# Genesis-Embodied-AI/ThinShellLab

Hardware: AMD Instinct MI355X
Metric: element-steps/s (fwd+adjoint), 100k-tri cloth; 1/2/4/8-GPU scaling (higher is better)
Workload: dtype f64

## Files before the change

### thinshelllab_amd/context.py

```python
import ctypes as C
import os

import numpy as np
import torch

from . import _lib
from ._lib import Body, ClothDesc, ContactPair, ElasticDesc, SceneDesc, SolveStats, StepStats, check


def _np(a, dt):
    return np.ascontiguousarray(a, dtype=dt)


def _ptr(t):
    if t is None:
        return None
    if isinstance(t, torch.Tensor):
        assert t.is_contiguous(), "tensor must be contiguous"
        return C.c_void_p(t.data_ptr())
    return C.c_void_p(t.ctypes.data)


def scene_desc(*, tot_NV, dt, mass, gravity, frozen, cloths=(), elastics=(), faces=None, bodies=(), pairs=(),
               k_contact=1000.0, eps_contact=1e-3, eps_v=0.01, damping=1.0, max_n_constraints=10000, grid_h=0.003, device=None):
# ... 591 lines not shown
        check(self.L.tsl_profile_read_events(self.h, C.byref(ev)), "tsl_profile_read_events")
        return dict(ms_per_launch=ms.value, launches=n.value, bytes_per_launch=b.value, ms_per_launch_events=ev.value)

    def bench_direct(self, cls, reps=20):
        out = (C.c_double * 4)()
        check(self.L.tsl_bench_direct(self.h, int(cls), int(reps), out), "tsl_bench_direct")
        return dict(us_per_launch=out[0], flops_per_launch=out[1], bytes_per_launch=out[2], launches=int(out[3]))

    def direct_info(self):
        out = (C.c_double * 10)()
        check(self.L.tsl_direct_info(self.h, out), "tsl_direct_info")
        keys = ("plans", "factorizations", "applications", "perturbed_pivots", "plan_seconds", "supernodes", "levels", "batches", "flops_per_factorization", "front_bytes")
        return dict(zip(keys, [float(v) for v in out]))

    def direct_counters(self):
        out = (C.c_double * 13)()
        check(self.L.tsl_direct_counters(self.h, out, 13), "tsl_direct_counters")
        keys = ("flow_launches", "flow_aborts", "plan_cache_hits", "panel_bytes", "schur_bytes", "g_bytes", "schur_entries", "plans_parked",
                "berr_seen", "berr_accepted", "berr_max", "berr_rel_max", "tiles_guarded")
        return dict(zip(keys, [float(v) for v in out]))

    def bench_spmv(self, variant=20, reps=500):
        us = C.c_double(0)
        check(self.L.tsl_bench_spmv(self.h, int(variant), int(reps), C.byref(us)), "tsl_bench_spmv")
        return us.value
```

### thinshelllab_amd/csrc/direct_host.hpp

```cpp
#pragma once
#include <array>
#include <chrono>

#include "k_direct.hpp"
#include "tsl_ctx.hpp"

#include <cerrno>
#include <fcntl.h>
#include <sys/file.h>
#include <sys/stat.h>
#include <unistd.h>
static void ds_flow_token_acquire(DirectSolver& d) {
  char bus[64] = "dev";
  if (hipDeviceGetPCIBusId(bus, sizeof(bus), d.device) != hipSuccess) { (void)hipGetLastError(); snprintf(bus, sizeof(bus), "dev%d", d.device); }
  for (char* q = bus; *q; q++) if (*q == ':' || *q == '/') *q = '_';
  d.flow_token = -1; d.flow_token_asked = d.n_factor;
  for (const char* dir : {"/dev/shm", "/tmp"}) {
    const std::string path = std::string(dir) + "/tsl_flow_" + bus;
    int fd = open(path.c_str(), O_RDWR | O_CLOEXEC);
    if (fd < 0 && errno == ENOENT) {
      fd = open(path.c_str(), O_CREAT | O_RDWR | O_CLOEXEC, 0666);
      if (fd < 0 && (errno == ENOENT || errno == ENOTDIR)) continue;
      if (fd < 0 && errno == EEXIST) fd = open(path.c_str(), O_RDWR | O_CLOEXEC);
    } else if (fd < 0 && errno == ENOTDIR) continue;
// ... 9 lines not shown
  d.flow_token_fd = -1; d.flow_token = 0;
}
static bool ds_flow_token_held(DirectSolver& d) {
  if (d.token_lender) return ds_flow_token_held(*d.token_lender);
  if (d.flow_token == 0 || (d.flow_token < 0 && d.n_factor - d.flow_token_asked >= 256)) ds_flow_token_acquire(d);
  return d.flow_token > 0;
}

static inline int ds_nblk(long n, int b) { return (int)((n + b - 1) / b); }

static inline bool ds_use_small(const DirectSolver& d, const DsBatch& b) {
  if (b.max_pp > DS_SMALL) return false;
  return (size_t)b.count <= (size_t)d.plan.n_cu * ds_small_per_cu(b.max_pp) * (size_t)d.small_rounds;
}

static void ds_launch_gemm(hipStream_t s, const DsDev& D, const DsBatch& b, int mode, int ds_xcd_map, int ds_g32_below = 0, int part = 0, int max_lead = 0) {
  const int rows = mode == 0 ? b.max_pp : b.max_bp, cols = b.max_bp;
  const dim3 grid((cols + 63) / 64, (rows + 63) / 64, b.count);
  const long tiles = (long)grid.x * grid.y * grid.z;
  const int ta = (max_lead + 63) / 64;
  if (part == 1 && ta == 0) return;
  if (mode == 1 && part != 0) {
    hipLaunchKernelGGL((k_ds_gemm<1, 4>), part == 1 ? dim3(ta, ta, b.count) : grid, dim3(256), 0, s, D, b.first, part);
    return;
  }
  if (mode == 0 && ds_g32_below > 0 && tiles < ds_g32_below) {
    hipLaunchKernelGGL(k_ds_gemm_g32, dim3(part == 1 ? 2 * ta : (cols + 31) / 32, (rows + 31) / 32, b.count), dim3(256), 0, s, D, b.first, part);
    return;
  }
  if (mode == 0 && part != 0) {
    hipLaunchKernelGGL((k_ds_gemm<0, 4>), part == 1 ? dim3(ta, grid.y, b.count) : grid, dim3(256), 0, s, D, b.first, part);
    return;
  }
  if (ds_xcd_map > 0 && b.count >= ds_xcd_map) {
    const int gx = grid.x, gy = grid.y, nf = b.count;
    const long ng = ((long)nf + 7) / 8 * 8 * gx * gy;
    if (mode == 0) hipLaunchKernelGGL((k_ds_gemm_x<0, 4>), dim3((unsigned)ng), dim3(256), 0, s, D, b.first, gx, gy, nf);
    else hipLaunchKernelGGL((k_ds_gemm_x<1, 4>), dim3((unsigned)ng), dim3(256), 0, s, D, b.first, gx, gy, nf);
    return;
  }
  if (mode == 0) hipLaunchKernelGGL((k_ds_gemm<0, 4>), grid, dim3(256), 0, s, D, b.first, 0);
  else hipLaunchKernelGGL((k_ds_gemm<1, 4>), grid, dim3(256), 0, s, D, b.first, 0);
}
static void ds_launch_extend(hipStream_t s, const DsDev& D, int lv0, int nf, int max_ld, int part = 0, int max_span = 0) {
  const int xspan = part == 1 ? 64 * DS_XU : DS_XSPAN;
  const int nsp = ((part == 0 ? max_ld : max_span) + xspan - 1) / xspan;
  if (nsp <= 0) return;
  hipLaunchKernelGGL(k_ds_extend_panels, dim3(((max_ld / 3 + 2 + 3) / 4) * nsp, nf), dim3(256), 0, s, D, lv0, nsp, part, xspan);
}
static void ds_launch_level_start(tsl_ctx* c, hipStream_t s, const DsDev& D, int l, int part = 0, const DsBatch* b = nullptr) {
  DirectSolver& d = c->ds;
  const DirectPlan& P = d.plan;
  const int lv0 = P.level_ptr[l], nf = P.level_ptr[l + 1] - lv0;
  if (l > 0) ds_launch_extend(s, D, lv0, nf, P.level_maxld[l], part, part == 0 ? 0 : part == 1 ? b->max_pp : std::max(b->max_bp, b->max_pp));
  const int i0 = part == 2 ? P.blk_lmid[l] : P.blk_lptr[l], i1 = part == 1 ? P.blk_lmid[l] : P.blk_lptr[l + 1];
  const int nb = i1 - i0, npad = part == 2 ? 0 : nf;
  const long nt = (long)nb * 9 + (long)npad * DS_T;
  if (nt > 0)
    hipLaunchKernelGGL(k_ds_assemble_level, dim3(ds_nblk(nt, 256)), dim3(256), 0, s, i0, nb, (const int*)d.blk_q.p, (const double*)c->vals.p, (const long long*)d.blk_dst.p,
                       (const int*)d.blk_ld.p, lv0, npad, d.frl.p, d.arena.p, l == 0 ? 1 : 0);
  if (c->nc > 0) {
    const int g0 = part == 2 ? P.cgr_lmid[l] : P.cgr_lptr[l], g1 = part == 1 ? P.cgr_lmid[l] : P.cgr_lptr[l + 1];
    const int ng = g1 - g0;
    if (ng > 0) hipLaunchKernelGGL(k_ds_assemble_contacts_level, dim3(ds_nblk((long)ng * 64, 256)), dim3(256), 0, s, g0, ng, (const int*)d.cgr_ptr.p, (const int*)d.cgr_ent.p,
                                   (const long long*)d.cgr_dst.p, (const int*)d.cgr_ld.p, (const double*)c->c_H.p, d.arena.p);
  }
}


static long ds_flow_wgs(const DirectPlan& P, const DsBatch& b) {
  long n = 0;
  for (int z = 0; z < b.count; z++) { const long ns = (P.fr[P.level_sn[b.first + z]].pp / DS_T + DS_FLOW_B - 1) / DS_FLOW_B; n += ns * ns; }
  return n;
}
static bool ds_flow_eligible(DirectSolver& d, const DirectPlan& P, const DsBatch& b, hipStream_t s) {
  if (!d.flow || b.count > DS_FLOW_MAXF || b.max_pp < 2 * DS_T) return false;
  { hipStreamCaptureStatus cs = hipStreamCaptureStatusNone;
    if (hipStreamIsCapturing(s, &cs) != hipSuccess || cs != hipStreamCaptureStatusNone) return false; }
  if (!ds_flow_token_held(d)) return false;
  if (ds_use_small(d, b) && !(d.flow & 2)) return false;
  if (d.flow_cap == 0) {
    int occ = 0, dev = 0;
    hipDeviceProp_t prop;
// ... 325 lines not shown
static int direct_factor(tsl_ctx* c, int stop_sn = -1, const char* dump_path = nullptr, const double* eager_r = nullptr, double* eager_z = nullptr) {
  DirectSolver& d = c->ds;
  hipStream_t s = c->stream;
  TSL_TRY(direct_plan(c));
  if (d.numeric_valid) return 0;
  d.eager_n = 0;
  const DirectPlan& P = d.plan;
  const DsDev D = ds_dev(c);
  if (d.prezero_pending) {
    HIP_OK(hipStreamWaitEvent(s, d.ev_zero, 0));
    d.prezero_pending = false;
    if (P.leaf_ranges.empty() && d.prezero_n < (size_t)P.arena_leaf) HIP_OK(hipMemsetAsync(d.arena.p + d.prezero_n, 0, ((size_t)P.arena_leaf - d.prezero_n) * sizeof(double), s));
  } else if (P.leaf_ranges.empty()) HIP_OK(hipMemsetAsync(d.arena.p, 0, (size_t)P.arena_leaf * sizeof(double), s));
  else for (const auto& r : P.leaf_ranges) HIP_OK(hipMemsetAsync(d.arena.p + r.first, 0, (size_t)r.second * sizeof(double), s));
  HIP_OK(hipMemsetAsync(d.bad.p, 0, 8 * sizeof(int), s));
  bool swept_at_root = false;
  int flow_wgs_sent = 0;
  auto invert_batch = [&](const DsBatch& b, hipStream_t bs, bool& flow_free) {
    const int lv0 = b.first, nf = b.count;
    const int tp = b.max_pp / DS_T;
    bool flowed = false;
    {
      const std::vector<DsBatch> pieces = ds_flow_pieces(d, P, b, flow_free, bs);
      std::vector<DsFlowArgs> fas(pieces.size());
      bool ready = !pieces.empty();
      for (size_t i = 0; ready && i < pieces.size(); i++) ready = ds_flow_prepare(d, P, pieces[i], true, fas[i], bs);
      if (ready) {
        for (size_t i = 0; i < pieces.size(); i++) { ds_flow_launch(bs, D, pieces[i].first, fas[i], d); d.n_flow++; flow_wgs_sent += fas[i].tile0[fas[i].nf]; }
        flowed = true; flow_free = false;
      }
// ... 57 lines not shown
        const int c0 = std::min((d.lookahead >> 2) & 7, top - 2);
        const int c1r = (d.lookahead >> 5) & 15, c1 = c1r == 0 ? top - 1 : std::min(std::max(c1r, c0), top - 1);
        const int stage = lvl - (top - 2);
        const int lo = stage == 0 ? 0 : stage == 1 ? c0 : c1, hi = stage == 0 ? c0 : stage == 1 ? c1 : (c1r == 0 ? c1 : top);
        if (hi > lo && lo == d.eager_n && (stage > 0 || P.la_from < lvl)) {
          hipLaunchKernelGGL(k_ds_flow_gate, dim3(1), dim3(64), 0, ls, (const int*)(d.bad.p + DS_FLOW_ARRIVE), flow_wgs_sent);
          for (int l = lo; l < hi; l++) ds_sweep_up_level(ls, D, d, l, eager_r, eager_z);
          d.eager_n = hi; d.eager_r = eager_r; d.eager_z = eager_z;
          if (stage == 2) { HIP_OK(hipEventRecord(d.ev_la[LA_DRAIN], ls)); swept_at_root = true; }
        }
      }
      if (la_in) HIP_OK(hipStreamWaitEvent(s, d.ev_la[LA_REST], 0));
      if (b.max_bp > 0 && be < P.batches.size()) {
        int max_lead = 0;
        for (int q = 0; q < b.count; q++) max_lead = std::max(max_lead, P.fr[P.level_sn[b.first + q]].lead);
        HIP_OK(hipEventRecord(d.ev_la[LA_W], s));
        ds_launch_gemm(s, D, b, 0, 0, d.g32_below, 1, max_lead);
        HIP_OK(hipEventRecord(d.ev_la[LA_GA], s));
        ds_launch_gemm(s, D, b, 1, 0, 0, 1, max_lead);
        HIP_OK(hipEventRecord(d.ev_la[LA_A], s));
        HIP_OK(hipStreamWaitEvent(ls, d.ev_la[LA_W], 0));
        ds_launch_gemm(ls, D, b, 0, 0, d.g32_below, 2, max_lead);
        HIP_OK(hipStreamWaitEvent(ls, d.ev_la[LA_GA], 0));
        ds_launch_gemm(ls, D, b, 1, 0, 0, 2, max_lead);
      } else if (b.max_bp > 0) {
        ds_launch_gemm(s, D, b, 0, d.xcd_map, d.g32_below);
        ds_launch_gemm(s, D, b, 1, d.xcd_map);
      }
      bi = be;
      continue;
    }
    if (stop_here) {
      const DsFrontDesc& f = P.fr[stop_sn];
      std::vector<double> h((size_t)f.pp * f.ld);
// ... 217 lines not shown
```

### thinshelllab_amd/csrc/k_direct.hpp

```cpp
#pragma once
#include "direct_plan.hpp"
#include "tsl_device.hpp"

typedef double ds_d4 __attribute__((ext_vector_type(4)));

struct DsDev {
  const DsFrontDesc* fr;
  const DsFrontDesc* frl;
  const int* level_sn;
  double* A;
  double* S;
  double* G;
  double* scr;
  double* Y;
  const DsChildRec* ch;
  const int* pmap;
  const int* vtx;
  int* bad;
  double piv_tol;
  int dbg;
  unsigned long long* tlog;
};

__global__ void k_ds_rownorm(int NV, const int* __restrict__ slice_off, const int* __restrict__ slice_len, const double* __restrict__ vals, double* out) {
// ... 26 lines not shown
  if (t < (long)nblk * 9) {
    const long i = i0 + t / 9;
    const int e = (int)(t % 9);
    double* a = &A[dst[i] + (long long)(e / 3) * dld[i] + e % 3];
    const double v = vals[(size_t)src[i] + 64 * e];
    *a = cleared ? 0.0 + v : *a + v;
    return;
  }
  t -= (long)nblk * 9;
  if (t < (long)nf * DS_T) {
    const DsFrontDesc f = frl[lv0 + t / DS_T];
    const int i = f.p + (int)(t % DS_T);
    if (i < f.pp) A[f.off + (long long)i * f.ld + i] = 1.0;
  }
}
__global__ void __launch_bounds__(256) k_ds_assemble_contacts_level(int g0, int ng, const int* __restrict__ gptr, const int* __restrict__ gent, const long long* __restrict__ gdst,
                                                                    const int* __restrict__ gld, const double* __restrict__ H, double* __restrict__ A) {
  const int gi = (int)((blockIdx.x * (size_t)blockDim.x + threadIdx.x) >> 6), lane = threadIdx.x & 63;
  if (gi >= ng) return;
  const int g = g0 + gi;
  double v[9] = {0, 0, 0, 0, 0, 0, 0, 0, 0};
  for (int k = gptr[g] + lane; k < gptr[g + 1]; k += 64) {
    const int x = gent[k], c = x >> 4, sub = x & 15;
    const double* Hb = H + (size_t)c * 144 + (3 * (sub >> 2)) * 12 + 3 * (sub & 3);
#pragma unroll
    for (int r = 0; r < 3; r++)
#pragma unroll
      for (int cc = 0; cc < 3; cc++) v[3 * r + cc] += Hb[12 * r + cc];
  }
#pragma unroll
  for (int e = 0; e < 9; e++) v[e] = wave_sum(v[e]);
  if (lane == 0) {
    double* dst = A + gdst[g];
    const int ld = gld[g];
#pragma unroll
    for (int r = 0; r < 3; r++)
#pragma unroll
      for (int cc = 0; cc < 3; cc++) dst[(long long)r * ld + cc] += v[3 * r + cc];
  }
}

#define DS_PB 4
#define DS_BADLOG 64
#define DS_BAD_NOTE (8 + 4 * DS_BADLOG)
#define DS_BAD_INTS (DS_BAD_NOTE + 8)
#define DS_REDO 6
// ... 785 lines not shown
            }
      }
    }
    __syncthreads();
  }
  for (int i = ty; i < pp; i += 32) {
#pragma unroll
    for (int a = 0; a < 4; a++)
#pragma unroll
      for (int b = 0; b < 4; b++) if (b < nt) A[(size_t)(i + 8 * a) * f.ld + tx + 32 * b] = M[(i + 8 * a) * ls + tx + 32 * b];
  }
}

#define DS_SK 32
#define DS_GMC 8
template <int mode, int WPC>
TSL_DEV void ds_gemm_tile(const DsDev& D, int lv0, int bx, int by, int bz, int part = 0) {
  constexpr int SA = DS_SK + 1, SB = 64 + 1;
  __shared__ double As[64 * SA];
  __shared__ double Bs[DS_SK * SB];
  const DsFrontDesc f = D.frl[lv0 + bz];
  const int Mr = mode == 0 ? f.pp : f.bp, Nc = f.bp, K = f.pp;
  const int I0 = by * 64, J0 = bx * 64;
  if (I0 >= Mr || J0 >= Nc) return;
  if (mode == 1 && part != 0 && ((I0 < f.lead && J0 < f.lead) != (part == 1))) return;
  if (mode == 0 && part != 0 && ((J0 < f.lead) != (part == 1))) return;
  const double* F = D.A + f.off;
  double* G = D.G + f.goff;
  const int ld = f.ld, pp = f.pp;
  const double* Am = mode == 0 ? F : D.A + f.off21;
// ... 13 lines not shown
  double pa[8], pb0[4], pb1[4];
  auto gload = [&](int k0) {
#pragma unroll
    for (int q = 0; q < 8; q++) {
      const int r = ty + 8 * q;
      pa[q] = (r < 32 || rows_hi) ? Am[(size_t)(I0 + r) * lda + k0 + tx] : 0.0;
    }
#pragma unroll
    for (int q = 0; q < 4; q++) {
      const int r = ty + 8 * q;
      pb0[q] = Bm[(size_t)(k0 + r) * ldb + J0 + tx];
      pb1[q] = cols_hi ? Bm[(size_t)(k0 + r) * ldb + J0 + 32 + tx] : 0.0;
    }
  };
  gload(0);
  constexpr int GMC = DS_GMC;
  __shared__ int s_map[mode == 1 ? GMC : 1][128];
  __shared__ long long s_soff[mode == 1 ? GMC : 1];
  __shared__ int s_cbp[mode == 1 ? GMC : 1];
  int pre[GMC / 2];
  auto map_load = [&](int q) {
    const int k = threadIdx.x & 127;
    const int idx = k < 64 ? I0 + k : J0 + k - 64;
    return idx < f.bp ? D.pmap[D.ch[f.ch_off + q].pmap_off + pp + idx] : -1;
  };
  if (mode == 1) {
#pragma unroll
    for (int h = 0; h < GMC / 2; h++) { const int q = 2 * h + (threadIdx.x >> 7); pre[h] = q < f.nchild ? map_load(q) : -1; }
  }
  for (int k0 = 0; k0 < K; k0 += DS_SK) {
#pragma unroll
    for (int q = 0; q < 8; q++) As[(ty + 8 * q) * SA + tx] = pa[q];
#pragma unroll
    for (int q = 0; q < 4; q++) { Bs[(ty + 8 * q) * SB + tx] = pb0[q]; Bs[(ty + 8 * q) * SB + tx + 32] = pb1[q]; }
    __syncthreads();
    if (k0 + DS_SK < K) gload(k0 + DS_SK);
#pragma unroll
    for (int kk = 0; kk < DS_SK / 4; kk++) {
      const double a0 = As[(32 * wi + lr) * SA + 4 * kk + lk], a1 = As[(32 * wi + 16 + lr) * SA + 4 * kk + lk];
      const double b0 = Bs[(4 * kk + lk) * SB + 32 * wj + lr], b1 = Bs[(4 * kk + lk) * SB + 32 * wj + 16 + lr];
      acc[0][0] = __builtin_amdgcn_mfma_f64_16x16x4f64(a0, b0, acc[0][0], 0, 0, 0);
      acc[0][1] = __builtin_amdgcn_mfma_f64_16x16x4f64(a0, b1, acc[0][1], 0, 0, 0);
      acc[1][0] = __builtin_amdgcn_mfma_f64_16x16x4f64(a1, b0, acc[1][0], 0, 0, 0);
      acc[1][1] = __builtin_amdgcn_mfma_f64_16x16x4f64(a1, b1, acc[1][1], 0, 0, 0);
    }
    __syncthreads();
  }
  if (mode == 0) {
#pragma unroll
    for (int a = 0; a < 2; a++)
#pragma unroll
      for (int b = 0; b < 2; b++)
#pragma unroll
        for (int r = 0; r < 4; r++) {
          const int row = I0 + 32 * wi + 16 * a + lk + 4 * r, col = J0 + 32 * wj + 16 * b + lr;
          if (row < Mr && col < Nc) G[(size_t)row * f.bp + col] = acc[a][b][r];
        }
    return;
  }
  if (f.parent < 0) return;
  double s22[2][2][4];
#pragma unroll
  for (int a = 0; a < 2; a++)
#pragma unroll
    for (int b = 0; b < 2; b++)
#pragma unroll
      for (int r = 0; r < 4; r++) s22[a][b][r] = -acc[a][b][r];
  const int row0 = I0 + 32 * wi + lk, col0 = J0 + 32 * wj + lr;
  for (int q0 = 0; q0 < f.nchild; q0 += GMC) {
    const int nq = min(GMC, f.nchild - q0);
    if (q0 > 0) __syncthreads();
#pragma unroll
    for (int h = 0; h < GMC / 2; h++) {
      const int q = 2 * h + (threadIdx.x >> 7);
      if (q < nq) s_map[q][threadIdx.x & 127] = q0 == 0 ? pre[h] : map_load(q0 + q);
    }
    if ((int)threadIdx.x < nq) { const DsChildRec c = D.ch[f.ch_off + q0 + threadIdx.x]; s_soff[threadIdx.x] = c.soff; s_cbp[threadIdx.x] = c.bp; }
    __syncthreads();
    for (int q = 0; q < nq; q++) {
      const double* Sc = D.S + s_soff[q];
      const int cbp = s_cbp[q];
      const int cj0 = s_map[q][64 + 32 * wj + lr], cj1 = s_map[q][64 + 32 * wj + 16 + lr];
      const int dj0 = max(cj0, 0), dj1 = max(cj1, 0);
      int ci[2][4];
      double v0[2][4], v1[2][4];
#pragma unroll
      for (int a = 0; a < 2; a++)
#pragma unroll
        for (int r = 0; r < 4; r++) ci[a][r] = s_map[q][32 * wi + 16 * a + lk + 4 * r];
#pragma unroll
      for (int a = 0; a < 2; a++)
#pragma unroll
        for (int r = 0; r < 4; r++) {
          const double* Srow = Sc + (size_t)max(ci[a][r], 0) * cbp;
          v0[a][r] = Srow[dj0]; v1[a][r] = Srow[dj1];
        }
#pragma unroll
      for (int a = 0; a < 2; a++)
#pragma unroll
        for (int r = 0; r < 4; r++) {
          s22[a][0][r] = (ci[a][r] >= 0 && cj0 >= 0) ? s22[a][0][r] + v0[a][r] : s22[a][0][r];
          s22[a][1][r] = (ci[a][r] >= 0 && cj1 >= 0) ? s22[a][1][r] + v1[a][r] : s22[a][1][r];
        }
    }
  }
  double* Sf = D.S + f.soff;
#pragma unroll
  for (int a = 0; a < 2; a++)
#pragma unroll
    for (int r = 0; r < 4; r++) {
      const int row = row0 + 16 * a + 4 * r;
      if (row >= f.b) continue;
#pragma unroll
      for (int b = 0; b < 2; b++) {
        const int col = col0 + 16 * b;
        if (col < f.b) Sf[(size_t)row * f.bp + col] = s22[a][b][r];
      }
    }
}

#define DS_XU 4
#define DS_XSPAN 1024
#define DS_XMAXC 64
__global__ void __launch_bounds__(256) k_ds_extend_panels(DsDev D, int lv0, int nsp, int part, int xspan) {
  const DsFrontDesc f = D.frl[lv0 + blockIdx.y];
  const int ib = blockIdx.x / nsp, sp = blockIdx.x - ib * nsp;
  const int lane = threadIdx.x & 63, w = __builtin_amdgcn_readfirstlane(threadIdx.x >> 6);
  const int g = 4 * ib + w, ng = f.nv_own + f.nv_bnd;
  if (g >= ng + 2) return;
  const bool top = g >= ng ? g == ng : g < f.nv_own;
  if (!top && part == 1) return;
  const int ncol = top ? f.ld : f.pp;
  const int cA = (top && part == 2) ? f.pp : 0, cB = (top && part == 1) ? f.pp : ncol;
// ... 129 lines not shown
  for (int r = 0; r < 4; r++) G[(size_t)(I0 + 16 * wi + lk + 4 * r) * f.bp + J0 + 16 * wj + lr] = acc[r];
}

template <int mode, int WPC>
__global__ void __launch_bounds__(256, WPC) k_ds_gemm(DsDev D, int lv0, int part) {
  ds_gemm_tile<mode, WPC>(D, lv0, blockIdx.x, blockIdx.y, blockIdx.z, part);
}

template <int mode, int WPC>
__global__ void __launch_bounds__(256, WPC) k_ds_gemm_x(DsDev D, int lv0, int gx, int gy, int nf) {
  const unsigned L = blockIdx.x, xcd = L & 7, k = L >> 3;
  const unsigned tpf = (unsigned)gx * gy;
  const unsigned bz = (k / tpf) * 8 + xcd, t = k % tpf;
  if (bz >= (unsigned)nf) return;
  ds_gemm_tile<mode, WPC>(D, lv0, t % gx, t / gx, bz);
}

#define DS_VCHUNK 2048
TSL_DEV double ds_child_sum(const DsDev& D, const DsFrontDesc& f, int d) {
  int ci[4];
#pragma unroll
  for (int q = 0; q < 4; q++) ci[q] = q < f.nchild ? D.pmap[f.cpm[q] + d] : -1;
  double y[4];
#pragma unroll
  for (int q = 0; q < 4; q++) y[q] = ci[q] >= 0 ? D.Y[f.cy[q] + ci[q]] : 0.0;
  double a = ((y[0] + y[1]) + y[2]) + y[3];
  for (int q = 4; q < f.nchild; q++) {
    const DsChildRec c = D.ch[f.ch_off + q];
    const int cq = D.pmap[c.pmap_off + d];
    if (cq >= 0) a += D.Y[c.yoff + cq];
// ... 94 lines not shown
```

### thinshelllab_amd/csrc/tsl_ctx.hpp

```cpp
#pragma once
#include <memory>
#include <hip/hip_runtime.h>
#include <stdint.h>

#include <algorithm>
#include <cmath>
#include <cstdio>
#include <cstring>
#include <string>
#include <vector>

#include "../../include/tsl_hip.h"
#include "collider_host.hpp"
#include "sphere_host.hpp"
#include "box_host.hpp"
#include "sdf_host.hpp"
#include "capsule_host.hpp"
#include "k_body.hpp"
#include "direct_plan.hpp"
#include "scene_tables.hpp"

#define TSL_SLICE 64

extern thread_local std::string g_tsl_err;
// ... 91 lines not shown
  int eager_n = 0; const double* eager_r = nullptr; double* eager_z = nullptr;
  int lookahead = 103;
  int device = 0;
  int flow_wgs_last = 0;
  int flow = 3, flow_cap = 0, flow_epoch = 0;
  int flow_token = 0, flow_token_fd = -1;
  long flow_token_asked = 0;
  int small_rounds = 2;
  int xcd_map = 64;
  long n_flow = 0, n_flow_abort = 0;
  DevBuf<double> flow_x;
  DevBuf<int> flow_f;
  DevBuf<unsigned long long> tlog;
  int gemv_wide_below = 300;
  int g32_below = 1100;
  bool cons_checked = false;
  double* h_anorm = nullptr;
  int bench_batch = -1;
  double piv_tol = 1e-11;
  int fallback_cap = 1000;
  int leaf = 64;
  bool static_ready = false, numeric_valid = false;
  bool have_factor = false;
  int dbg = 0;
  double berr_tol = 1e-12, berr_rel_cap = 50.0;
  long berr_seen = 0, berr_accepted = 0;
  double berr_max = 0, berr_rel_max = 0;
  int n_setup_fail = 0;
  std::vector<std::unique_ptr<DsPlanSlot>> cache;
  int cache_cap = 64, cache_mb = 1024;
// ... 300 lines not shown
```

### thinshelllab_amd/csrc/tsl_hip.hip

```cpp
#include <stdarg.h>
#include <cctype>
#include <chrono>
#include <mutex>

#include <array>
#include <map>

#include "k_cloth.hpp"
#include "k_contact.hpp"
#include "k_fem.hpp"
#include "k_mg.hpp"
#include "k_param.hpp"
#include "k_solver.hpp"
#include "param_keys.hpp"
#include "tsl_ctx.hpp"

thread_local std::string g_tsl_err;
int tsl_fail(const char* fmt, ...) {
  char buf[1024];
  va_list ap;
  va_start(ap, fmt);
  vsnprintf(buf, sizeof(buf), fmt, ap);
  va_end(ap);
  g_tsl_err = buf;
// ... 262 lines not shown
  else if (k == "adj_spd_pc") c->adj_spd_pc = (int)v;
  else if (k == "adj_clamp") c->adj_clamp = v;
  else if (k == "adj_clamp_angleref") c->adj_clamp_angleref = (int)v;
  else if (k == "verbose") c->verbose = (int)v;
  else if (k == "direct") { c->ds.enable = (int)v; c->ds.numeric_valid = false; c->ds.hard = false; }
  else if (k == "direct_berr") c->ds.berr_tol = v;
  else if (k == "direct_small_rounds") { c->ds.small_rounds = std::max(1, (int)v); c->ds.plan_valid = false; c->ds.numeric_valid = false; c->ds.cache.clear(); }
  else if (k == "tet_warm") c->tet_warm = (int)v;
  else if (k == "ds_dbg") c->ds.dbg = (int)v;
  else if (k == "ds_bench_batch") c->ds.bench_batch = (int)v;
  else if (k == "direct_flow") c->ds.flow = std::max(0, (int)v);
  else if (k == "direct_flow_token") { if (v == 0) ds_flow_token_release(c->ds); }
  else if (k == "direct_gemv_wide_below") c->ds.gemv_wide_below = std::max(0, (int)v);
  else if (k == "direct_g32_below") c->ds.g32_below = std::max(0, (int)v);
  else if (k == "direct_lookahead") c->ds.lookahead = (int)v;
  else if (k == "direct_piv_tol") { c->ds.piv_tol = v; c->ds.numeric_valid = false; }
  else if (k == "direct_leaf") { c->ds.leaf = std::max(4, (int)v); c->ds.static_ready = false; c->ds.plan_valid = false; c->ds.numeric_valid = false; }
  else if (k == "gmres_m") c->gmres_m = (int)v;
  else if (k == "body_inv") { c->bd_enable = (int)v; c->bd_valid = false; }
  else if (k == "mg") c->mg_enable = (int)v;
  else if (k == "mg_coarse_exact") { c->mg_coarse_exact = (int)v; c->mg_ops_valid = false; }
  else if (k == "mg_dense_nodes") { c->mg_dense_auto = v < 0; if (v >= 0) c->mg_dense_nodes = (int)v; c->mg_ops_valid = false; }
  else return set_indexed_param(c, key, v);
  return 0;
}

extern "C" int tsl_set_frozen(tsl_ctx* c, const int32_t* fr) {
  Scope scope(c);
  (void)hipStreamSynchronize(c->stream);
  c->h_frozen.assign(fr, fr + 3 * (size_t)c->NV);
// ... 1549 lines not shown
  if (stale) {
    for (int i = 0; i < n; i++) HIP_OK(hipStreamSynchronize(G->m[i]->stream));
    TSL_TRY(group_merge(G));
  }
  lap(2);
  {
    DirectSolver& gd = g->ds;
    const DirectSolver& d0 = G->m[0]->ds;
    for (int i = 1; i < n; i++) {
      const DirectSolver& di = G->m[i]->ds;
      if (di.piv_tol != d0.piv_tol || di.flow != d0.flow || di.g32_below != d0.g32_below || di.gemv_wide_below != d0.gemv_wide_below || di.small_rounds != d0.small_rounds)
        return tsl_fail("scene group: members 0 and %d differ in a parameter of the factorisation (direct_piv_tol / _flow / _g32_below / _gemv_wide_below / _small_rounds)", i);
    }
    if (gd.piv_tol != d0.piv_tol) gd.piv_tol = d0.piv_tol;
    gd.flow = G->flow_lost ? 0 : d0.flow; gd.g32_below = d0.g32_below; gd.gemv_wide_below = d0.gemv_wide_below; gd.small_rounds = d0.small_rounds * n; gd.xcd_map = d0.xcd_map;
    gd.prezero = d0.prezero; gd.dbg = d0.dbg;
  }
  ss.assign(n, tsl_solve_stats{});
  std::vector<char> okv(n, 1);
  for (int attempt = 0; attempt < 2; attempt++) {
    DirectSolver& gd = g->ds;
    for (int i = 0; i < n; i++) { HIP_OK(hipEventRecord(G->ev_m[i], G->m[i]->stream)); HIP_OK(hipStreamWaitEvent(g->stream, G->ev_m[i], 0)); }
    gd.numeric_valid = false;
    if (attempt > 0) {
      gd.have_factor = false;
      if (gd.prezero_pending) { HIP_OK(hipStreamWaitEvent(g->stream, gd.ev_zero, 0)); gd.prezero_pending = false; }
    }
    TSL_TRY(direct_factor(g));
    if (attempt == 0) for (int i = 0; i < n; i++) { DirectSolver& d = G->m[i]->ds; if (++d.anorm_age >= 64) d.anorm_valid = false; }
    lap(3);
    TSL_TRY(direct_apply(g, G->vb.p, G->vx.p));
// ... 241 lines not shown
  int bad[4] = {0, 0, 0, 0};
  if (d.bad.p) HIP_OK(hipMemcpy(bad, d.bad.p, sizeof(bad), hipMemcpyDeviceToHost));
  out10[0] = (double)d.n_plans; out10[1] = (double)d.n_factor; out10[2] = (double)d.n_apply; out10[3] = bad[1] + bad[2] + bad[3]; out10[4] = d.t_plan;
  out10[5] = d.plan_valid ? d.plan.sym.n_sn : 0; out10[6] = d.plan_valid ? d.plan.n_levels : 0; out10[7] = d.plan_valid ? (double)d.plan.batches.size() : 0;
  out10[8] = d.plan_valid ? d.plan.flops : 0; out10[9] = d.plan_valid ? 8.0 * (double)(d.plan.arena + d.plan.sarena) : 0;
  return 0;
}
extern "C" int tsl_direct_counters(tsl_ctx* c, double* out, int32_t n) {
  const DirectSolver& d = c->ds;
  double e = 0;
  if (d.plan_valid) for (const DsFrontDesc& f : d.plan.fr) e += (double)f.b * f.b;
  size_t parked = 0;
  for (const auto& sl : d.cache) parked += sl->used ? 1 : 0;
  int redo = 0;
  if (n > 12 && d.bad.p) { HIP_OK(hipStreamSynchronize(c->stream)); HIP_OK(hipMemcpy(&redo, d.bad.p + DS_REDO, sizeof(int), hipMemcpyDeviceToHost)); }
  const double v[13] = {(double)d.n_flow, (double)d.n_flow_abort, (double)d.n_plan_hits, d.plan_valid ? 8.0 * (double)d.plan.arena : 0.0, d.plan_valid ? 8.0 * (double)d.plan.sarena : 0.0,
                        d.plan_valid ? 8.0 * (double)d.plan.garena : 0.0, e, (double)parked, (double)d.berr_seen, (double)d.berr_accepted, d.berr_max, d.berr_rel_max, (double)redo};
  for (int i = 0; i < std::min<int>(n, 13); i++) out[i] = v[i];
  return 0;
}

extern "C" int tsl_spd_project(tsl_ctx* c, double* blocks, int32_t n, int32_t D) {
  Scope scope(c);
  if (D != 2 && D != 3 && D != 9) return tsl_fail("tsl_spd_project: D must be 2, 3 or 9");
  if (c->spd_literal && D == 3) hipLaunchKernelGGL(k_spd_batch_literal, dim3(nblk(n, 256)), dim3(256), 0, c->stream, blocks, n, D);
  else if (c->spd_literal && D == 9) hipLaunchKernelGGL(k_spd_batch_literal, dim3(nblk((long)n * 16, 256)), dim3(256), 0, c->stream, blocks, n, D);
  else hipLaunchKernelGGL(k_spd_batch, dim3(nblk(n, 64)), dim3(64), 0, c->stream, blocks, n, D);
  HIP_OK(hipStreamSynchronize(c->stream));
  return 0;
}

#include "adjoint_api.hpp"
```

Before: 525,100.

## Add deep-prefetch lead Schur GEMM kernel and optional contact group presum

Adds a dedicated k_ds_lead_schur kernel for the lookahead lead-part Schur update. It holds DEPTH (3 or 4) K-slabs of register prefetch and double-buffers LDS so global loads overlap the MFMA work. It is enabled by default with depth 4 when the solver is not merged, and the shared epilogue code is factored into helpers. It also adds an opt-in (off by default) path that precomputes contact group 3x3 sums once per factorization and then applies them per level. The deeper prefetch raises register and LDS pressure, which may lower occupancy.

```diff
diff --git a/thinshelllab_amd/context.py b/thinshelllab_amd/context.py
--- a/thinshelllab_amd/context.py
+++ b/thinshelllab_amd/context.py
@@ -629,10 +629,10 @@
         return dict(zip(keys, [float(v) for v in out]))
 
     def direct_counters(self):
-        out = (C.c_double * 13)()
-        check(self.L.tsl_direct_counters(self.h, out, 13), "tsl_direct_counters")
+        out = (C.c_double * 15)()
+        check(self.L.tsl_direct_counters(self.h, out, 15), "tsl_direct_counters")
         keys = ("flow_launches", "flow_aborts", "plan_cache_hits", "panel_bytes", "schur_bytes", "g_bytes", "schur_entries", "plans_parked",
-                "berr_seen", "berr_accepted", "berr_max", "berr_rel_max", "tiles_guarded")
+                "berr_seen", "berr_accepted", "berr_max", "berr_rel_max", "tiles_guarded", "lead_gemm_launches", "lead_gemm_min_slabs")
         return dict(zip(keys, [float(v) for v in out]))
 
     def bench_spmv(self, variant=20, reps=500):
diff --git a/thinshelllab_amd/csrc/direct_host.hpp b/thinshelllab_amd/csrc/direct_host.hpp
--- a/thinshelllab_amd/csrc/direct_host.hpp
+++ b/thinshelllab_amd/csrc/direct_host.hpp
@@ -47,33 +47,40 @@
   return (size_t)b.count <= (size_t)d.plan.n_cu * ds_small_per_cu(b.max_pp) * (size_t)d.small_rounds;
 }
 
-static void ds_launch_gemm(hipStream_t s, const DsDev& D, const DsBatch& b, int mode, int ds_xcd_map, int ds_g32_below = 0, int part = 0, int max_lead = 0) {
+static inline bool ds_lead_depth_ok(int v) { return v == 0 || v == 3 || v == 4; }
+static bool ds_launch_gemm(hipStream_t s, const DsDev& D, const DsBatch& b, int mode, int ds_xcd_map, int ds_g32_below = 0, int part = 0, int max_lead = 0, int lead_depth = 0) {
   const int rows = mode == 0 ? b.max_pp : b.max_bp, cols = b.max_bp;
   const dim3 grid((cols + 63) / 64, (rows + 63) / 64, b.count);
   const long tiles = (long)grid.x * grid.y * grid.z;
   const int ta = (max_lead + 63) / 64;
-  if (part == 1 && ta == 0) return;
+  if (part == 1 && ta == 0) return false;
+  if (mode == 1 && part == 1 && lead_depth > 0) {
+    if (lead_depth == 3) hipLaunchKernelGGL((k_ds_lead_schur<3>), dim3(ta, ta, b.count), dim3(256), 0, s, D, b.first);
+    else hipLaunchKernelGGL((k_ds_lead_schur<4>), dim3(ta, ta, b.count), dim3(256), 0, s, D, b.first);
+    return true;
+  }
   if (mode == 1 && part != 0) {
     hipLaunchKernelGGL((k_ds_gemm<1, 4>), part == 1 ? dim3(ta, ta, b.count) : grid, dim3(256), 0, s, D, b.first, part);
-    return;
+    return false;
   }
   if (mode == 0 && ds_g32_below > 0 && tiles < ds_g32_below) {
     hipLaunchKernelGGL(k_ds_gemm_g32, dim3(part == 1 ? 2 * ta : (cols + 31) / 32, (rows + 31) / 32, b.count), dim3(256), 0, s, D, b.first, part);
-    return;
+    return false;
   }
   if (mode == 0 && part != 0) {
     hipLaunchKernelGGL((k_ds_gemm<0, 4>), part == 1 ? dim3(ta, grid.y, b.count) : grid, dim3(256), 0, s, D, b.first, part);
-    return;
+    return false;
   }
   if (ds_xcd_map > 0 && b.count >= ds_xcd_map) {
     const int gx = grid.x, gy = grid.y, nf = b.count;
     const long ng = ((long)nf + 7) / 8 * 8 * gx * gy;
     if (mode == 0) hipLaunchKernelGGL((k_ds_gemm_x<0, 4>), dim3((unsigned)ng), dim3(256), 0, s, D, b.first, gx, gy, nf);
     else hipLaunchKernelGGL((k_ds_gemm_x<1, 4>), dim3((unsigned)ng), dim3(256), 0, s, D, b.first, gx, gy, nf);
-    return;
+    return false;
   }
   if (mode == 0) hipLaunchKernelGGL((k_ds_gemm<0, 4>), grid, dim3(256), 0, s, D, b.first, 0);
   else hipLaunchKernelGGL((k_ds_gemm<1, 4>), grid, dim3(256), 0, s, D, b.first, 0);
+  return false;
 }
 static void ds_launch_extend(hipStream_t s, const DsDev& D, int lv0, int nf, int max_ld, int part = 0, int max_span = 0) {
   const int xspan = part == 1 ? 64 * DS_XU : DS_XSPAN;
@@ -95,11 +102,22 @@
   if (c->nc > 0) {
     const int g0 = part == 2 ? P.cgr_lmid[l] : P.cgr_lptr[l], g1 = part == 1 ? P.cgr_lmid[l] : P.cgr_lptr[l + 1];
     const int ng = g1 - g0;
-    if (ng > 0) hipLaunchKernelGGL(k_ds_assemble_contacts_level, dim3(ds_nblk((long)ng * 64, 256)), dim3(256), 0, s, g0, ng, (const int*)d.cgr_ptr.p, (const int*)d.cgr_ent.p,
+    if (ng > 0 && d.contact_presum)
+      hipLaunchKernelGGL(k_ds_apply_contact_sums, dim3(ds_nblk((long)ng * 9, 256)), dim3(256), 0, s, g0, ng, (const long long*)d.cgr_dst.p, (const int*)d.cgr_ld.p, (const double*)d.cgr_sum.p, d.arena.p);
+    else if (ng > 0) hipLaunchKernelGGL(k_ds_assemble_contacts_level, dim3(ds_nblk((long)ng * 64, 256)), dim3(256), 0, s, g0, ng, (const int*)d.cgr_ptr.p, (const int*)d.cgr_ent.p,
                                    (const long long*)d.cgr_dst.p, (const int*)d.cgr_ld.p, (const double*)c->c_H.p, d.arena.p);
   }
 }
-
+static int ds_launch_contact_sums(tsl_ctx* c, hipStream_t s) {
+  DirectSolver& d = c->ds;
+  const DirectPlan& P = d.plan;
+  if (c->nc <= 0 || !d.contact_presum) return 0;
+  const int ng = P.cgr_lptr.size() > (size_t)P.n_levels ? P.cgr_lptr[P.n_levels] : 0;
+  if (ng <= 0) return 0;
+  if (d.cgr_sum.n < (size_t)9 * ng) { if (d.cgr_sum.alloc((size_t)9 * ng + (size_t)9 * ng / 4 + 144)) return -1; }
+  hipLaunchKernelGGL(k_ds_contact_group_sums, dim3(ds_nblk((long)ng * 64, 256)), dim3(256), 0, s, ng, (const int*)d.cgr_ptr.p, (const int*)d.cgr_ent.p, (const double*)c->c_H.p, d.cgr_sum.p);
+  return 0;
+}
 
 static long ds_flow_wgs(const DirectPlan& P, const DsBatch& b) {
   long n = 0;
@@ -455,6 +473,7 @@
   } else if (P.leaf_ranges.empty()) HIP_OK(hipMemsetAsync(d.arena.p, 0, (size_t)P.arena_leaf * sizeof(double), s));
   else for (const auto& r : P.leaf_ranges) HIP_OK(hipMemsetAsync(d.arena.p + r.first, 0, (size_t)r.second * sizeof(double), s));
   HIP_OK(hipMemsetAsync(d.bad.p, 0, 8 * sizeof(int), s));
+  TSL_TRY(ds_launch_contact_sums(c, s));
   bool swept_at_root = false;
   int flow_wgs_sent = 0;
   auto invert_batch = [&](const DsBatch& b, hipStream_t bs, bool& flow_free) {
@@ -542,10 +561,16 @@
       if (b.max_bp > 0 && be < P.batches.size()) {
         int max_lead = 0;
         for (int q = 0; q < b.count; q++) max_lead = std::max(max_lead, P.fr[P.level_sn[b.first + q]].lead);
+        const int depth = d.merged ? 0 : d.lead_depth;
+        int n_lead = 0;
         HIP_OK(hipEventRecord(d.ev_la[LA_W], s));
-        ds_launch_gemm(s, D, b, 0, 0, d.g32_below, 1, max_lead);
+        n_lead += ds_launch_gemm(s, D, b, 0, 0, d.g32_below, 1, max_lead, depth) ? 1 : 0;
         HIP_OK(hipEventRecord(d.ev_la[LA_GA], s));
-        ds_launch_gemm(s, D, b, 1, 0, 0, 1, max_lead);
+        n_lead += ds_launch_gemm(s, D, b, 1, 0, 0, 1, max_lead, depth) ? 1 : 0;
+        if (n_lead > 0) {
+          d.n_lead_gemm += n_lead;
+          for (int q = 0; q < b.count; q++) { const int ns = P.fr[P.level_sn[b.first + q]].pp / DS_SK; d.lead_min_slabs = d.lead_min_slabs == 0 ? ns : std::min(d.lead_min_slabs, ns); }
+        }
         HIP_OK(hipEventRecord(d.ev_la[LA_A], s));
         HIP_OK(hipStreamWaitEvent(ls, d.ev_la[LA_W], 0));
         ds_launch_gemm(ls, D, b, 0, 0, d.g32_below, 2, max_lead);
diff --git a/thinshelllab_amd/csrc/k_direct.hpp b/thinshelllab_amd/csrc/k_direct.hpp
--- a/thinshelllab_amd/csrc/k_direct.hpp
+++ b/thinshelllab_amd/csrc/k_direct.hpp
@@ -64,22 +64,43 @@
     if (i < f.pp) A[f.off + (long long)i * f.ld + i] = 1.0;
   }
 }
+TSL_DEV void ds_contact_group_sum(int g, int lane, const int* __restrict__ gptr, const int* __restrict__ gent, const double* __restrict__ H, double (&v)[9]) {
+#pragma unroll
+  for (int e = 0; e < 9; e++) v[e] = 0.0;
+  for (int k = gptr[g] + lane; k < gptr[g + 1]; k += 64) {
+    const int x = gent[k], c = x >> 4, sub = x & 15;
+    const double* Hb = H + (size_t)c * 144 + (3 * (sub >> 2)) * 12 + 3 * (sub & 3);
+#pragma unroll
+    for (int r = 0; r < 3; r++)
+#pragma unroll
+      for (int cc = 0; cc < 3; cc++) v[3 * r + cc] += Hb[12 * r + cc];
+  }
+#pragma unroll
+  for (int e = 0; e < 9; e++) v[e] = wave_sum(v[e]);
+}
+__global__ void __launch_bounds__(256) k_ds_contact_group_sums(int ng, const int* __restrict__ gptr, const int* __restrict__ gent, const double* __restrict__ H, double* __restrict__ sums) {
+  const int g = (int)((blockIdx.x * (size_t)blockDim.x + threadIdx.x) >> 6), lane = threadIdx.x & 63;
+  if (g >= ng) return;
+  double v[9];
+  ds_contact_group_sum(g, lane, gptr, gent, H, v);
+  if (lane == 0) {
+#pragma unroll
+    for (int e = 0; e < 9; e++) sums[(size_t)9 * g + e] = v[e];
+  }
+}
+__global__ void __launch_bounds__(256) k_ds_apply_contact_sums(int g0, int ng, const long long* __restrict__ gdst, const int* __restrict__ gld, const double* __restrict__ sums, double* __restrict__ A) {
+  const long t = (long)blockIdx.x * blockDim.x + threadIdx.x;
+  if (t >= (long)ng * 9) return;
+  const int g = g0 + (int)(t / 9), e = (int)(t % 9);
+  A[gdst[g] + (long long)(e / 3) * gld[g] + e % 3] += sums[(size_t)9 * g + e];
+}
 __global__ void __launch_bounds__(256) k_ds_assemble_contacts_level(int g0, int ng, const int* __restrict__ gptr, const int* __restrict__ gent, const long long* __restrict__ gdst,
                                                                     const int* __restrict__ gld, const double* __restrict__ H, double* __restrict__ A) {
   const int gi = (int)((blockIdx.x * (size_t)blockDim.x + threadIdx.x) >> 6), lane = threadIdx.x & 63;
   if (gi >= ng) return;
   const int g = g0 + gi;
-  double v[9] = {0, 0, 0, 0, 0, 0, 0, 0, 0};
-  for (int k = gptr[g] + lane; k < gptr[g + 1]; k += 64) {
-    const int x = gent[k], c = x >> 4, sub = x & 15;
-    const double* Hb = H + (size_t)c * 144 + (3 * (sub >> 2)) * 12 + 3 * (sub & 3);
-#pragma unroll
-    for (int r = 0; r < 3; r++)
-#pragma unroll
-      for (int cc = 0; cc < 3; cc++) v[3 * r + cc] += Hb[12 * r + cc];
-  }
-#pragma unroll
-  for (int e = 0; e < 9; e++) v[e] = wave_sum(v[e]);
+  double v[9];
+  ds_contact_group_sum(g, lane, gptr, gent, H, v);
   if (lane == 0) {
     double* dst = A + gdst[g];
     const int ld = gld[g];
@@ -895,6 +916,94 @@
 
 #define DS_SK 32
 #define DS_GMC 8
+TSL_DEV void ds_g_store(const DsFrontDesc& f, double* G, int I0, int J0, const ds_d4 (&acc)[2][2]) {
+  const int lane = threadIdx.x & 63, w = threadIdx.x >> 6, wi = w >> 1, wj = w & 1, lr = lane & 15, lk = lane >> 4;
+#pragma unroll
+  for (int a = 0; a < 2; a++)
+#pragma unroll
+    for (int b = 0; b < 2; b++)
+#pragma unroll
+      for (int r = 0; r < 4; r++) {
+        const int row = I0 + 32 * wi + 16 * a + lk + 4 * r, col = J0 + 32 * wj + 16 * b + lr;
+        if (row < f.pp && col < f.bp) G[(size_t)row * f.bp + col] = acc[a][b][r];
+      }
+}
+TSL_DEV int ds_schur_map_load(const DsDev& D, const DsFrontDesc& f, int I0, int J0, int q) {
+  const int k = threadIdx.x & 127;
+  const int idx = k < 64 ? I0 + k : J0 + k - 64;
+  return idx < f.bp ? D.pmap[D.ch[f.ch_off + q].pmap_off + f.pp + idx] : -1;
+}
+TSL_DEV void ds_schur_prefetch(const DsDev& D, const DsFrontDesc& f, int I0, int J0, int (&pre)[DS_GMC / 2]) {
+#pragma unroll
+  for (int h = 0; h < DS_GMC / 2; h++) { const int q = 2 * h + (threadIdx.x >> 7); pre[h] = q < f.nchild ? ds_schur_map_load(D, f, I0, J0, q) : -1; }
+}
+TSL_DEV void ds_schur_epilogue(const DsDev& D, const DsFrontDesc& f, int I0, int J0, const ds_d4 (&acc)[2][2], const int (&pre)[DS_GMC / 2]) {
+  constexpr int GMC = DS_GMC;
+  __shared__ int s_map[GMC][128];
+  __shared__ long long s_soff[GMC];
+  __shared__ int s_cbp[GMC];
+  if (f.parent < 0) return;
+  const int lane = threadIdx.x & 63, w = threadIdx.x >> 6, wi = w >> 1, wj = w & 1, lr = lane & 15, lk = lane >> 4;
+  double s22[2][2][4];
+#pragma unroll
+  for (int a = 0; a < 2; a++)
+#pragma unroll
+    for (int b = 0; b < 2; b++)
+#pragma unroll
+      for (int r = 0; r < 4; r++) s22[a][b][r] = -acc[a][b][r];
+  const int row0 = I0 + 32 * wi + lk, col0 = J0 + 32 * wj + lr;
+  for (int q0 = 0; q0 < f.nchild; q0 += GMC) {
+    const int nq = min(GMC, f.nchild - q0);
+    if (q0 > 0) __syncthreads();
+#pragma unroll
+    for (int h = 0; h < GMC / 2; h++) {
+      const int q = 2 * h + (threadIdx.x >> 7);
+      if (q < nq) s_map[q][threadIdx.x & 127] = q0 == 0 ? pre[h] : ds_schur_map_load(D, f, I0, J0, q0 + q);
+    }
+    if ((int)threadIdx.x < nq) { const DsChildRec c = D.ch[f.ch_off + q0 + threadIdx.x]; s_soff[threadIdx.x] = c.soff; s_cbp[threadIdx.x] = c.bp; }
+    __syncthreads();
+    for (int q = 0; q < nq; q++) {
+      const double* Sc = D.S + s_soff[q];
+      const int cbp = s_cbp[q];
+      const int cj0 = s_map[q][64 + 32 * wj + lr], cj1 = s_map[q][64 + 32 * wj + 16 + lr];
+      const int dj0 = max(cj0, 0), dj1 = max(cj1, 0);
+      int ci[2][4];
+      double v0[2][4], v1[2][4];
+#pragma unroll
+      for (int a = 0; a < 2; a++)
+#pragma unroll
+        for (int r = 0; r < 4; r++) ci[a][r] = s_map[q][32 * wi + 16 * a + lk + 4 * r];
+#pragma unroll
+      for (int a = 0; a < 2; a++)
+#pragma unroll
+        for (int r = 0; r < 4; r++) {
+          const double* Srow = Sc + (size_t)max(ci[a][r], 0) * cbp;
+          v0[a][r] = Srow[dj0]; v1[a][r] = Srow[dj1];
+        }
+#pragma unroll
+      for (int a = 0; a < 2; a++)
+#pragma unroll
+        for (int r = 0; r < 4; r++) {
+          s22[a][0][r] = (ci[a][r] >= 0 && cj0 >= 0) ? s22[a][0][r] + v0[a][r] : s22[a][0][r];
+          s22[a][1][r] = (ci[a][r] >= 0 && cj1 >= 0) ? s22[a][1][r] + v1[a][r] : s22[a][1][r];
+        }
+    }
+  }
+  double* Sf = D.S + f.soff;
+#pragma unroll
+  for (int a = 0; a < 2; a++)
+#pragma unroll
+    for (int r = 0; r < 4; r++) {
+      const int row = row0 + 16 * a + 4 * r;
+      if (row >= f.b) continue;
+#pragma unroll
+      for (int b = 0; b < 2; b++) {
+        const int col = col0 + 16 * b;
+        if (col < f.b) Sf[(size_t)row * f.bp + col] = s22[a][b][r];
+      }
+    }
+}
+
 template <int mode, int WPC>
 TSL_DEV void ds_gemm_tile(const DsDev& D, int lv0, int bx, int by, int bz, int part = 0) {
   constexpr int SA = DS_SK + 1, SB = 64 + 1;
@@ -938,20 +1047,8 @@
     }
   };
   gload(0);
-  constexpr int GMC = DS_GMC;
-  __shared__ int s_map[mode == 1 ? GMC : 1][128];
-  __shared__ long long s_soff[mode == 1 ? GMC : 1];
-  __shared__ int s_cbp[mode == 1 ? GMC : 1];
-  int pre[GMC / 2];
-  auto map_load = [&](int q) {
-    const int k = threadIdx.x & 127;
-    const int idx = k < 64 ? I0 + k : J0 + k - 64;
-    return idx < f.bp ? D.pmap[D.ch[f.ch_off + q].pmap_off + pp + idx] : -1;
-  };
-  if (mode == 1) {
-#pragma unroll
-    for (int h = 0; h < GMC / 2; h++) { const int q = 2 * h + (threadIdx.x >> 7); pre[h] = q < f.nchild ? map_load(q) : -1; }
-  }
+  int pre[DS_GMC / 2];
+  if constexpr (mode == 1) ds_schur_prefetch(D, f, I0, J0, pre);
   for (int k0 = 0; k0 < K; k0 += DS_SK) {
 #pragma unroll
     for (int q = 0; q < 8; q++) As[(ty + 8 * q) * SA + tx] = pa[q];
@@ -970,77 +1067,8 @@
     }
     __syncthreads();
   }
-  if (mode == 0) {
-#pragma unroll
-    for (int a = 0; a < 2; a++)
-#pragma unroll
-      for (int b = 0; b < 2; b++)
-#pragma unroll
-        for (int r = 0; r < 4; r++) {
-          const int row = I0 + 32 * wi + 16 * a + lk + 4 * r, col = J0 + 32 * wj + 16 * b + lr;
-          if (row < Mr && col < Nc) G[(size_t)row * f.bp + col] = acc[a][b][r];
-        }
-    return;
-  }
-  if (f.parent < 0) return;
-  double s22[2][2][4];
-#pragma unroll
-  for (int a = 0; a < 2; a++)
-#pragma unroll
-    for (int b = 0; b < 2; b++)
-#pragma unroll
-      for (int r = 0; r < 4; r++) s22[a][b][r] = -acc[a][b][r];
-  const int row0 = I0 + 32 * wi + lk, col0 = J0 + 32 * wj + lr;
-  for (int q0 = 0; q0 < f.nchild; q0 += GMC) {
-    const int nq = min(GMC, f.nchild - q0);
-    if (q0 > 0) __syncthreads();
-#pragma unroll
-    for (int h = 0; h < GMC / 2; h++) {
-      const int q = 2 * h + (threadIdx.x >> 7);
-      if (q < nq) s_map[q][threadIdx.x & 127] = q0 == 0 ? pre[h] : map_load(q0 + q);
-    }
-    if ((int)threadIdx.x < nq) { const DsChildRec c = D.ch[f.ch_off + q0 + threadIdx.x]; s_soff[threadIdx.x] = c.soff; s_cbp[threadIdx.x] = c.bp; }
-    __syncthreads();
-    for (int q = 0; q < nq; q++) {
-      const double* Sc = D.S + s_soff[q];
-      const int cbp = s_cbp[q];
-      const int cj0 = s_map[q][64 + 32 * wj + lr], cj1 = s_map[q][64 + 32 * wj + 16 + lr];
-      const int dj0 = max(cj0, 0), dj1 = max(cj1, 0);
-      int ci[2][4];
-      double v0[2][4], v1[2][4];
-#pragma unroll
-      for (int a = 0; a < 2; a++)
-#pragma unroll
-        for (int r = 0; r < 4; r++) ci[a][r] = s_map[q][32 * wi + 16 * a + lk + 4 * r];
-#pragma unroll
-      for (int a = 0; a < 2; a++)
-#pragma unroll
-        for (int r = 0; r < 4; r++) {
-          const double* Srow = Sc + (size_t)max(ci[a][r], 0) * cbp;
-          v0[a][r] = Srow[dj0]; v1[a][r] = Srow[dj1];
-        }
-#pragma unroll
-      for (int a = 0; a < 2; a++)
-#pragma unroll
-        for (int r = 0; r < 4; r++) {
-          s22[a][0][r] = (ci[a][r] >= 0 && cj0 >= 0) ? s22[a][0][r] + v0[a][r] : s22[a][0][r];
-          s22[a][1][r] = (ci[a][r] >= 0 && cj1 >= 0) ? s22[a][1][r] + v1[a][r] : s22[a][1][r];
-        }
-    }
-  }
-  double* Sf = D.S + f.soff;
-#pragma unroll
-  for (int a = 0; a < 2; a++)
-#pragma unroll
-    for (int r = 0; r < 4; r++) {
-      const int row = row0 + 16 * a + 4 * r;
-      if (row >= f.b) continue;
-#pragma unroll
-      for (int b = 0; b < 2; b++) {
-        const int col = col0 + 16 * b;
-        if (col < f.b) Sf[(size_t)row * f.bp + col] = s22[a][b][r];
-      }
-    }
+  if constexpr (mode == 0) ds_g_store(f, G, I0, J0, acc);
+  else ds_schur_epilogue(D, f, I0, J0, acc, pre);
 }
 
 #define DS_XU 4
@@ -1200,6 +1228,76 @@
   const unsigned bz = (k / tpf) * 8 + xcd, t = k % tpf;
   if (bz >= (unsigned)nf) return;
   ds_gemm_tile<mode, WPC>(D, lv0, t % gx, t / gx, bz);
+}
+
+template <int DEPTH>
+__global__ void __launch_bounds__(256, 2) k_ds_lead_schur(DsDev D, int lv0) {
+  constexpr int SA = DS_SK + 1, SB = 64 + 1;
+  __shared__ double As[2][64 * SA];
+  __shared__ double Bs[2][DS_SK * SB];
+  const DsFrontDesc f = D.frl[lv0 + blockIdx.z];
+  const int Mr = f.bp, Nc = f.bp, K = f.pp;
+  const int I0 = blockIdx.y * 64, J0 = blockIdx.x * 64;
+  if (I0 >= Mr || J0 >= Nc) return;
+  if (!(I0 < f.lead && J0 < f.lead)) return;
+  const double* Am = D.A + f.off21;
+  const double* Bm = D.G + f.goff;
+  const int lda = f.pp, ldb = f.bp;
+  const int lane = threadIdx.x & 63, w = threadIdx.x >> 6, wi = w >> 1, wj = w & 1, lr = lane & 15, lk = lane >> 4;
+  const bool rows_hi = I0 + 32 < Mr, cols_hi = J0 + 32 < Nc;
+  ds_d4 acc[2][2];
+#pragma unroll
+  for (int a = 0; a < 2; a++)
+#pragma unroll
+    for (int b = 0; b < 2; b++) acc[a][b] = ds_d4{0.0, 0.0, 0.0, 0.0};
+  const int tx = threadIdx.x & 31, ty = threadIdx.x >> 5;
+  double pa[DEPTH][8], pb0[DEPTH][4], pb1[DEPTH][4];
+  auto gload = [&](double (&a8)[8], double (&b0)[4], double (&b1)[4], int k0) {
+#pragma unroll
+    for (int q = 0; q < 8; q++) {
+      const int r = ty + 8 * q;
+      a8[q] = (r < 32 || rows_hi) ? Am[(size_t)(I0 + r) * lda + k0 + tx] : 0.0;
+    }
+#pragma unroll
+    for (int q = 0; q < 4; q++) {
+      const int r = ty + 8 * q;
+      b0[q] = Bm[(size_t)(k0 + r) * ldb + J0 + tx];
+      b1[q] = cols_hi ? Bm[(size_t)(k0 + r) * ldb + J0 + 32 + tx] : 0.0;
+    }
+  };
+#pragma unroll
+  for (int d = 0; d < DEPTH; d++)
+    if (d * DS_SK < K) gload(pa[d], pb0[d], pb1[d], d * DS_SK);
+  int pre[DS_GMC / 2];
+  ds_schur_prefetch(D, f, I0, J0, pre);
+  int cur = 0;
+  for (int kb = 0; kb < K; kb += DEPTH * DS_SK) {
+#pragma unroll
+    for (int d = 0; d < DEPTH; d++) {
+      const int k0 = kb + d * DS_SK;
+      if (k0 < K) {
+        double* as = As[cur];
+        double* bs = Bs[cur];
+#pragma unroll
+        for (int q = 0; q < 8; q++) as[(ty + 8 * q) * SA + tx] = pa[d][q];
+#pragma unroll
+        for (int q = 0; q < 4; q++) { bs[(ty + 8 * q) * SB + tx] = pb0[d][q]; bs[(ty + 8 * q) * SB + tx + 32] = pb1[d][q]; }
+        __syncthreads();
+        if (k0 + DEPTH * DS_SK < K) gload(pa[d], pb0[d], pb1[d], k0 + DEPTH * DS_SK);
+#pragma unroll
+        for (int kk = 0; kk < DS_SK / 4; kk++) {
+          const double a0 = as[(32 * wi + lr) * SA + 4 * kk + lk], a1 = as[(32 * wi + 16 + lr) * SA + 4 * kk + lk];
+          const double b0 = bs[(4 * kk + lk) * SB + 32 * wj + lr], b1 = bs[(4 * kk + lk) * SB + 32 * wj + 16 + lr];
+          acc[0][0] = __builtin_amdgcn_mfma_f64_16x16x4f64(a0, b0, acc[0][0], 0, 0, 0);
+          acc[0][1] = __builtin_amdgcn_mfma_f64_16x16x4f64(a0, b1, acc[0][1], 0, 0, 0);
+          acc[1][0] = __builtin_amdgcn_mfma_f64_16x16x4f64(a1, b0, acc[1][0], 0, 0, 0);
+          acc[1][1] = __builtin_amdgcn_mfma_f64_16x16x4f64(a1, b1, acc[1][1], 0, 0, 0);
+        }
+        cur ^= 1;
+      }
+    }
+  }
+  ds_schur_epilogue(D, f, I0, J0, acc, pre);
 }
 
 #define DS_VCHUNK 2048
diff --git a/thinshelllab_amd/csrc/tsl_ctx.hpp b/thinshelllab_amd/csrc/tsl_ctx.hpp
--- a/thinshelllab_amd/csrc/tsl_ctx.hpp
+++ b/thinshelllab_amd/csrc/tsl_ctx.hpp
@@ -129,6 +129,11 @@
   DevBuf<unsigned long long> tlog;
   int gemv_wide_below = 300;
   int g32_below = 1100;
+  int lead_depth = 4;
+  long n_lead_gemm = 0;
+  int lead_min_slabs = 0;
+  int contact_presum = 0;
+  DevBuf<double> cgr_sum;
   bool cons_checked = false;
   double* h_anorm = nullptr;
   int bench_batch = -1;
diff --git a/thinshelllab_amd/csrc/tsl_hip.hip b/thinshelllab_amd/csrc/tsl_hip.hip
--- a/thinshelllab_amd/csrc/tsl_hip.hip
+++ b/thinshelllab_amd/csrc/tsl_hip.hip
@@ -300,6 +300,14 @@
   else if (k == "direct_gemv_wide_below") c->ds.gemv_wide_below = std::max(0, (int)v);
   else if (k == "direct_g32_below") c->ds.g32_below = std::max(0, (int)v);
   else if (k == "direct_lookahead") c->ds.lookahead = (int)v;
+  else if (k == "direct_lead_depth") {
+    if (!ds_lead_depth_ok((int)v) || v != (int)v) return tsl_fail("tsl_set_param: direct_lead_depth must be 0, 3 or 4 (got %g)", v);
+    c->ds.lead_depth = (int)v;
+  }
+  else if (k == "direct_contact_presum") {
+    if (v != 0.0 && v != 1.0) return tsl_fail("tsl_set_param: direct_contact_presum must be 0 or 1 (got %g)", v);
+    c->ds.contact_presum = (int)v; c->ds.numeric_valid = false;
+  }
   else if (k == "direct_piv_tol") { c->ds.piv_tol = v; c->ds.numeric_valid = false; }
   else if (k == "direct_leaf") { c->ds.leaf = std::max(4, (int)v); c->ds.static_ready = false; c->ds.plan_valid = false; c->ds.numeric_valid = false; }
   else if (k == "gmres_m") c->gmres_m = (int)v;
@@ -1879,7 +1887,7 @@
     }
     if (gd.piv_tol != d0.piv_tol) gd.piv_tol = d0.piv_tol;
     gd.flow = G->flow_lost ? 0 : d0.flow; gd.g32_below = d0.g32_below; gd.gemv_wide_below = d0.gemv_wide_below; gd.small_rounds = d0.small_rounds * n; gd.xcd_map = d0.xcd_map;
-    gd.prezero = d0.prezero; gd.dbg = d0.dbg;
+    gd.prezero = d0.prezero; gd.dbg = d0.dbg; gd.contact_presum = d0.contact_presum;
   }
   ss.assign(n, tsl_solve_stats{});
   std::vector<char> okv(n, 1);
@@ -2151,9 +2159,10 @@
   for (const auto& sl : d.cache) parked += sl->used ? 1 : 0;
   int redo = 0;
   if (n > 12 && d.bad.p) { HIP_OK(hipStreamSynchronize(c->stream)); HIP_OK(hipMemcpy(&redo, d.bad.p + DS_REDO, sizeof(int), hipMemcpyDeviceToHost)); }
-  const double v[13] = {(double)d.n_flow, (double)d.n_flow_abort, (double)d.n_plan_hits, d.plan_valid ? 8.0 * (double)d.plan.arena : 0.0, d.plan_valid ? 8.0 * (double)d.plan.sarena : 0.0,
-                        d.plan_valid ? 8.0 * (double)d.plan.garena : 0.0, e, (double)parked, (double)d.berr_seen, (double)d.berr_accepted, d.berr_max, d.berr_rel_max, (double)redo};
-  for (int i = 0; i < std::min<int>(n, 13); i++) out[i] = v[i];
+  const double v[15] = {(double)d.n_flow, (double)d.n_flow_abort, (double)d.n_plan_hits, d.plan_valid ? 8.0 * (double)d.plan.arena : 0.0, d.plan_valid ? 8.0 * (double)d.plan.sarena : 0.0,
+                        d.plan_valid ? 8.0 * (double)d.plan.garena : 0.0, e, (double)parked, (double)d.berr_seen, (double)d.berr_accepted, d.berr_max, d.berr_rel_max, (double)redo,
+                        (double)d.n_lead_gemm, (double)d.lead_min_slabs};
+  for (int i = 0; i < std::min<int>(n, 15); i++) out[i] = v[i];
   return 0;
 }
 
```

After: 520,700. About the same (-0.8%).
